# 0xMiden/miden-vm

Measured on AMD Instinct MI355X. Metric: trace rows/sec proved (2^20-row trace, 96-bit sec), higher is better.
Workload: dtype u64 (Goldilocks field, p = 2^64 - 2^32 + 1); 1 GPU; full proof of miden:20:51:8 (DummyMidenAir 2^20 x 51 + 8 EF aux), 96-bit production PCS params (blowup 8, FRI arity 4, 27 queries, PoW 4/12/16), Poseidon2 LMCS; trace resident in HBM, transcript on host; log_trace_rows=20, main_width=51, aux_width_ef=8, log_blowup=3, proof_bytes=137697, parallelism=1 GPU

## Files before the change

miden-vm_amd/csrc/deep.hip:

```cpp
#include "gl.cuh"
#include "kernels.hpp"

__global__ __launch_bounds__(256) void k_bary_weights(const u64* tw, int log_n, u64 g, e2 y0, e2 y1, u64* w0, u64* w1) {
  const size_t n = (size_t)1 << log_n;
  const size_t base = (size_t)blockIdx.x * 1024 + threadIdx.x;
  const size_t half = n >> 1;
  u64 xs[4], nrm[8], pre[8];
  e2 den[8];
#pragma unroll
  for (int k = 0; k < 4; k++) {
    size_t r = base + (size_t)k * 256;
    u64 x = 0;
    if (r < n) x = gl_mul(g, half ? (r < half ? tw[r] : gl_neg(tw[r - half])) : 1);
    xs[k] = x;
    den[2 * k] = e2_sub(y0, e2_make(x));
    den[2 * k + 1] = e2_sub(y1, e2_make(x));
  }
  u64 run = 1;
#pragma unroll
  for (int k = 0; k < 8; k++) {
    nrm[k] = gl_sub(gl_sqr(den[k].c0), gl_mul7(gl_sqr(den[k].c1)));
    pre[k] = run;
    run = gl_mul(run, nrm[k]);
  }
  u64 inv = gl_inv(run);
#pragma unroll
  for (int k = 7; k >= 0; k--) {
    u64 ni = gl_mul(inv, pre[k]);
    inv = gl_mul(inv, nrm[k]);
    size_t r = base + (size_t)(k >> 1) * 256;
    if (r < n) {
      u64 s = gl_mul(ni, xs[k >> 1]);
      u64* w = (k & 1) ? w1 : w0;
      w[2 * r] = gl_mul(den[k].c0, s);
      w[2 * r + 1] = gl_mul(gl_neg(den[k].c1), s);
    }
  }
}

static constexpr int OOD_ROWS_PER_BLOCK = 8192;
__global__ __launch_bounds__(256) void k_ood_partial(const u64* lde, int log_n, int log_blowup, const u64* w0, const u64* w1,
                                                     u64* partial, unsigned chunks) {
  __shared__ u64 red[4][256];
  const size_t n = (size_t)1 << log_n;
  const size_t col = blockIdx.y, chunk = blockIdx.x;
  const u64* f = lde + ((col << log_blowup) << log_n);
  const size_t r0 = chunk * OOD_ROWS_PER_BLOCK;
  const size_t r1 = r0 + OOD_ROWS_PER_BLOCK < n ? r0 + OOD_ROWS_PER_BLOCK : n;
  e2 a0 = e2_make(0), a1 = e2_make(0);
  for (size_t r = r0 + threadIdx.x; r < r1; r += 256) {
    u64 v = f[r];
    a0 = e2_add(a0, e2_mulf(e2{w0[2 * r], w0[2 * r + 1]}, v));
    a1 = e2_add(a1, e2_mulf(e2{w1[2 * r], w1[2 * r + 1]}, v));
  }
  red[0][threadIdx.x] = a0.c0; red[1][threadIdx.x] = a0.c1; red[2][threadIdx.x] = a1.c0; red[3][threadIdx.x] = a1.c1;
  __syncthreads();
  for (int s = 128; s > 0; s >>= 1) {
    if ((int)threadIdx.x < s) {
#pragma unroll
      for (int k = 0; k < 4; k++) red[k][threadIdx.x] = gl_add(red[k][threadIdx.x], red[k][threadIdx.x + s]);
    }
    __syncthreads();
  }
  if (threadIdx.x < 4) partial[(col * chunks + chunk) * 4 + threadIdx.x] = red[threadIdx.x][0];
}

void deep_ood_eval_batch(mh_ctx* c, std::vector<OodJob>& jobs, int log_blowup) {
  struct Weights {
    int log_n;
    size_t coset0;
    e2 y0, y1;
    DevBuf w0, w1;
  };
  std::vector<std::unique_ptr<Weights>> weights;
  struct Slot {
    size_t off = 0, ncol = 0;
    unsigned chunks = 0;
  };
  std::vector<Slot> slots(jobs.size());
  size_t total = 0;
  for (size_t k = 0; k < jobs.size(); k++) {
    OodJob& j = jobs[k];
    const LdeMatrix& m = *j.m;
    if (j.col_end > m.width) j.col_end = m.width;
    j.out0.assign(m.width, e2_make(0));
    j.out1.assign(m.width, e2_make(0));
    if (j.col_begin >= j.col_end) continue;
    const size_t n = (size_t)1 << m.log_n;
    slots[k].ncol = j.col_end - j.col_begin;
    slots[k].chunks = (unsigned)((n + OOD_ROWS_PER_BLOCK - 1) / OOD_ROWS_PER_BLOCK);
    slots[k].off = total;
    total += slots[k].ncol * slots[k].chunks * 4;
  }
  if (!total) return;
  DevBuf partial(total * 8), one;
  for (size_t k = 0; k < jobs.size(); k++) {
    if (!slots[k].ncol) continue;
    const OodJob& j = jobs[k];
    const LdeMatrix& m = *j.m;
    const int log_n = m.log_n;
    const size_t n = (size_t)1 << log_n;
    const u64 g = gl_mul(gl_lde_shift(log_n + log_blowup), gl_pow(gl_two_adic_generator(log_n + log_blowup), m.coset0));
    const u64* tw = log_n ? c->twiddles(log_n, false) : nullptr;
    if (!tw) {
      if (!one.p) {
        one.alloc(8);
        u64 v = 1;
        c->h2d(one.p, &v, 8);
      }
      tw = one.u();
    }
    ProfScope ps(c, "deep_ood_eval", (double)n * 8.0 * slots[k].ncol + 64.0 * n);
    Weights* w = nullptr;
    for (auto& cand : weights)
      if (cand->log_n == log_n && cand->coset0 == m.coset0 && e2_eq(cand->y0, j.y0) && e2_eq(cand->y1, j.y1)) w = cand.get();
    if (!w) {
      weights.emplace_back(new Weights{log_n, m.coset0, j.y0, j.y1, DevBuf(n * 16), DevBuf(n * 16)});
      w = weights.back().get();
      MH_LAUNCH(k_bary_weights, dim3((unsigned)((n + 1023) / 1024)), dim3(256), 0, c->stream, tw, log_n, g, j.y0, j.y1, w->w0.u(), w->w1.u());
    }
    MH_LAUNCH(k_ood_partial, dim3(slots[k].chunks, (unsigned)slots[k].ncol), dim3(256), 0, c->stream,
              m.lde.u() + ((j.col_begin << m.log_cosets) << log_n), log_n, m.log_cosets, w->w0.u(), w->w1.u(), partial.u() + slots[k].off,
              slots[k].chunks);
  }
  std::vector<u64> host(total);
  c->d2h(host.data(), partial.p, total * 8);
  for (size_t k = 0; k < jobs.size(); k++) {
    if (!slots[k].ncol) continue;
    OodJob& j = jobs[k];
    const LdeMatrix& m = *j.m;
    const int log_n = m.log_n;
    const size_t n = (size_t)1 << log_n;
    const u64 g = gl_mul(gl_lde_shift(log_n + log_blowup), gl_pow(gl_two_adic_generator(log_n + log_blowup), m.coset0));
    const u64 g_inv = gl_inv(g), n_inv = gl_inv((u64)n % GL_P);
    const e2 s0 = e2_mulf(e2_sub(e2_exp_pow2(e2_mulf(j.y0, g_inv), log_n), e2_make(1)), n_inv);
    const e2 s1 = e2_mulf(e2_sub(e2_exp_pow2(e2_mulf(j.y1, g_inv), log_n), e2_make(1)), n_inv);
    for (size_t col = 0; col < slots[k].ncol; col++) {
      e2 a0 = e2_make(0), a1 = e2_make(0);
      for (unsigned ch = 0; ch < slots[k].chunks; ch++) {
        const u64* p = host.data() + slots[k].off + (col * slots[k].chunks + ch) * 4;
        a0 = e2_add(a0, e2{p[0], p[1]});
        a1 = e2_add(a1, e2{p[2], p[3]});
      }
      j.out0[j.col_begin + col] = e2_mul(a0, s0);
      j.out1[j.col_begin + col] = e2_mul(a1, s1);
    }
  }
}
void deep_ood_eval_matrix(mh_ctx* c, const LdeMatrix& m, int log_blowup, e2 y0, e2 y1, std::vector<e2>& out0, std::vector<e2>& out1,
                          size_t col_begin, size_t col_end) {
  std::vector<OodJob> jobs(1);
  jobs[0].m = &m; jobs[0].y0 = y0; jobs[0].y1 = y1; jobs[0].col_begin = col_begin; jobs[0].col_end = col_end;
  deep_ood_eval_batch(c, jobs, log_blowup);
  out0.swap(jobs[0].out0);
  out1.swap(jobs[0].out1);
}

static constexpr int DEEP_MAX_MATS = 128;
static constexpr unsigned DEEP_FLUSH = 128;
#ifndef DEEP_UNROLL
#define DEEP_UNROLL 2
#endif
#ifndef DEEP_PTS_N
#define DEEP_PTS_N 1
#endif
static constexpr int DEEP_PTS = DEEP_PTS_N;
struct DeepMat {
  const u64* lde;
  u32 width, coef_off;
  int log_n;
};
struct DeepArgs {
  DeepMat m[DEEP_MAX_MATS];
  int n_mats, log_n, log_blowup;
  const u64* negc;
  const u64* tw;
  const u64* coset_x;
  e2 z0, z1, fred0, fred1, beta;
  u64* out;
};

template <bool PLANES>
__global__ __launch_bounds__(256) void k_deep_assemble(DeepArgs a) {
  const size_t N = (size_t)1 << a.log_n;
  const size_t j = blockIdx.y;
  const size_t base = (size_t)blockIdx.x * (256 * DEEP_PTS) + threadIdx.x;
  size_t r[DEEP_PTS];
#pragma unroll
  for (int k = 0; k < DEEP_PTS; k++) r[k] = base + (size_t)k * 256;
  e2 neg[DEEP_PTS];
  u64 w[DEEP_PTS][2][6];
#pragma unroll
  for (int k = 0; k < DEEP_PTS; k++) {
    neg[k] = e2_make(0);
#pragma unroll
    for (int e = 0; e < 2; e++)
#pragma unroll
      for (int i = 0; i < 6; i++) w[k][e][i] = 0;
  }
  auto flush = [&]() {
    const u64 C[6] = {1ULL, 1ULL << 22, 1ULL << 44, 1ULL << 32, 1ULL << 54, GL_EPS << 12};
#pragma unroll
    for (int k = 0; k < DEEP_PTS; k++) {
      u64 s0 = w[k][0][0], s1 = w[k][1][0];
#pragma unroll
      for (int i = 1; i < 6; i++) {
        s0 = gl_add(s0, gl_mul(w[k][0][i], C[i]));
        s1 = gl_add(s1, gl_mul(w[k][1][i], C[i]));
      }
      neg[k] = e2_add(neg[k], e2{s0, s1});
#pragma unroll
      for (int e = 0; e < 2; e++)
#pragma unroll
        for (int i = 0; i < 6; i++) w[k][e][i] = 0;
    }
  };
  u32 pending = 0;
#pragma unroll 1
  for (int mi = 0; mi < a.n_mats; mi++) {
    const DeepMat m = a.m[mi];
    const size_t nm_mask = ((size_t)1 << m.log_n) - 1;
    const u64* colp = m.lde + (j << m.log_n);
    const size_t cstride = (size_t)1 << (m.log_n + a.log_blowup);
#pragma unroll DEEP_UNROLL
    for (u32 cidx = 0; cidx < m.width; cidx++) {
      const u64 cf0 = a.negc[2 * (m.coef_off + cidx)], cf1 = a.negc[2 * (m.coef_off + cidx) + 1];
      u32 al[2][3];
#pragma unroll
      for (int i = 0; i < 3; i++) {
        al[0][i] = (u32)(cf0 >> (22 * i)) & 0x3FFFFFu;
        al[1][i] = (u32)(cf1 >> (22 * i)) & 0x3FFFFFu;
      }
#pragma unroll
      for (int k = 0; k < DEEP_PTS; k++) {
        if (r[k] < N) {
          const u64 v = colp[r[k] & nm_mask];
          const u32 v0 = (u32)v, v1 = (u32)(v >> 32);
#pragma unroll
          for (int e = 0; e < 2; e++) {
            w[k][e][0] += (u64)al[e][0] * v0;
            w[k][e][1] += (u64)al[e][1] * v0;
            w[k][e][2] += (u64)al[e][2] * v0;
            w[k][e][3] += (u64)al[e][0] * v1;
            w[k][e][4] += (u64)al[e][1] * v1;
            w[k][e][5] += (u64)al[e][2] * v1;
          }
        }
      }
      colp += cstride;
      if (++pending == DEEP_FLUSH) {
        flush();
        pending = 0;
      }
    }
  }
  flush();
  const size_t half = N >> 1;
  const u64 cx = a.coset_x[j];
  e2 den[2 * DEEP_PTS];
  u64 nrm[2 * DEEP_PTS], pre[2 * DEEP_PTS];
#pragma unroll
  for (int k = 0; k < DEEP_PTS; k++) {
    u64 x = 0;
    if (r[k] < N) x = gl_mul(cx, half ? (r[k] < half ? a.tw[r[k]] : gl_neg(a.tw[r[k] - half])) : 1);
    den[2 * k] = e2_sub(a.z0, e2_make(x));
    den[2 * k + 1] = e2_sub(a.z1, e2_make(x));
  }
  u64 run = 1;
#pragma unroll
  for (int k = 0; k < 2 * DEEP_PTS; k++) {
    nrm[k] = gl_sub(gl_sqr(den[k].c0), gl_mul7(gl_sqr(den[k].c1)));
    pre[k] = run;
    run = gl_mul(run, nrm[k]);
  }
  u64 inv = gl_inv(run);
  e2 qinv[2 * DEEP_PTS];
#pragma unroll
  for (int k = 2 * DEEP_PTS - 1; k >= 0; k--) {
    u64 ni = gl_mul(inv, pre[k]);
// ... 85 lines not shown
```

miden-vm_amd/csrc/ntt.hip:

```cpp
#include "ctx.hpp"
#include "gl.cuh"
#include "kernels.hpp"
#include "poseidon2_fast.cuh"
#include <utility>

#ifndef NTT_ASM_MUL
#define NTT_ASM_MUL 2
#endif
#if P2F_ASM && NTT_ASM_MUL == 1
#define NTT_MUL1 p2f_mul
#elif P2F_ASM && NTT_ASM_MUL == 2
#define NTT_MUL1 p2f_mul_nv
#else
#define NTT_MUL1 p2f_mul_c
#endif

static constexpr int NTT_TILE_LOG = 12;
static constexpr int NTT_TILE_LOG_BIG = 14;
static constexpr int NTT_THREADS = 256;
static int ntt_tile_log(int log_n) {
  static const int big_max = [] {
    const char* e = getenv("MH_NTT_BIG_MAX");
    return e ? atoi(e) : 22;
  }();
  return log_n > 20 && log_n <= big_max ? NTT_TILE_LOG_BIG : NTT_TILE_LOG;
}

static bool ntt_coef_rot(int log_n) {
  static const int on = [] { const char* e = getenv("MH_NTT_ROT"); return e ? atoi(e) : 1; }();
  return on && log_n >= NTT_TILE_LOG && ntt_tile_log(log_n) == NTT_TILE_LOG;
}

struct PowTable {
  u64 pw[32];
};
__global__ void k_fill_powers(u64* out, size_t n, PowTable t, u64 scale) {
  size_t k = blockIdx.x * (size_t)blockDim.x + threadIdx.x;
  if (k >= n) return;
  u64 r = scale;
  size_t e = k;
#pragma unroll 1
  for (int i = 0; e; i++, e >>= 1)
    if (e & 1) r = gl_mul(r, t.pw[i]);
  out[k] = r;
}

static void fill_powers(mh_ctx* c, u64* out, size_t n, u64 base, u64 scale) {
  PowTable t;
  u64 b = base;
  for (int i = 0; i < 32; i++) {
    t.pw[i] = b;
    b = gl_sqr(b);
  }
  if (n == 0) return;
  MH_LAUNCH(k_fill_powers, dim3((n + 255) / 256), dim3(256), 0, c->stream, out, n, t, scale);
}

const u64* mh_ctx::twiddles(int log_n, bool inverse) {
  auto& m = inverse ? tw_inv : tw_fwd;
  auto it = m.find(log_n);
  if (it != m.end()) return it->second.u();
  size_t half = log_n ? ((size_t)1 << (log_n - 1)) : 1;
  DevBuf b(half * 8);
  u64 w = gl_two_adic_generator(log_n);
  if (inverse) w = gl_inv(w);
  fill_powers(this, b.u(), half, w, 1);
  const u64* p = b.u();
  m[log_n] = std::move(b);
  return p;
}

__global__ __launch_bounds__(256) void k_transpose_rm_to_cm(const u64* __restrict__ in, u64* __restrict__ out, size_t n,
                                                           size_t w) {
  __shared__ u64 tile[32][33];
  size_t r0 = (size_t)blockIdx.x * 32, c0 = (size_t)blockIdx.y * 32;
  int tx = threadIdx.x & 31, ty = threadIdx.x >> 5;
  for (int k = ty; k < 32; k += 8) {
    size_t r = r0 + k, cc = c0 + tx;
    if (r < n && cc < w) tile[k][tx] = in[r * w + cc];
  }
  __syncthreads();
  for (int k = ty; k < 32; k += 8) {
    size_t cc = c0 + k, r = r0 + tx;
    if (r < n && cc < w) out[cc * n + r] = gl_canon(tile[tx][k]);
  }
}

void launch_transpose_rm_to_cm(mh_ctx* c, const u64* in, u64* out, size_t n, size_t w, hipStream_t stream) {
  dim3 grid((unsigned)((n + 31) / 32), (unsigned)((w + 31) / 32));
  MH_LAUNCH(k_transpose_rm_to_cm, grid, dim3(256), 0, stream ? stream : c->stream, in, out, n, w);
}

struct NttPassArgs {
  const u64* src;
  u64* dst;
  size_t src_col_stride, dst_col_stride, dst_z_stride;
  int log_n, s_lo, r_bits, cb;
  int dif;
  int canon_out;
  const u64* tw_round[4];
  const u64* scale_lo;
  const u64* scale_hi;
  int lb;
  size_t scale_lo_z, scale_hi_z;
  u32 n_z;
  const u64* scale_full;
  int col_fastest;
  size_t src_z_stride;
  int rot;
  int direct_first;
  u32 group_cols, group_z;
  const u64* step;
};

#if defined(__HIP_DEVICE_COMPILE__)
__device__ __forceinline__ u64 ntt_canon(u64 t) {
  const u64 u = t + GL_EPS;
  return u < t ? u : t;
}
__device__ __forceinline__ u64 ntt_add(u64 a, u64 t) {
  u64 s = a + t;
  s += (s < t) ? GL_EPS : 0;
  return s;
}
__device__ __forceinline__ u64 ntt_sub(u64 a, u64 t) {
  u64 d = a - t;
  d -= (a < t) ? GL_EPS : 0;
  return d;
}
__device__ __forceinline__ u64 ntt_mul_pow2(u64 x, int S) {
  const int q = S >> 5, r = S & 31;
  const u64 y01 = x << r;
  const u32 y2 = r ? (u32)(hi32(x) >> (32 - r)) : 0u;
  if (q == 0) {
    u64 v = (u64)y2 * 0xFFFFFFFFu + y01;
    v += (v < y01) ? GL_EPS : 0;
    return v;
  }
  if (q == 1) {
    const u64 a0 = (u64)lo32(y01) << 32;
    u64 v = (u64)hi32(y01) * 0xFFFFFFFFu + a0;
    v += (v < a0) ? GL_EPS : 0;
    u64 w = v - y2;
    w -= (v < (u64)y2) ? GL_EPS : 0;
    return w;
  }
  const u64 v = (u64)lo32(y01) * 0xFFFFFFFFu;
  const u64 b = ((u64)y2 << 32) | hi32(y01);
  u64 w = v - b;
  w -= (v < b) ? GL_EPS : 0;
  return w;
}
__device__ __forceinline__ void ntt_bfly_dit(u64& a, u64& b, int E) {
  const u64 t = ntt_canon(E % 96 ? ntt_mul_pow2(b, E % 96) : b);
  const u64 s = ntt_add(a, t), d = ntt_sub(a, t);
  if (E >= 96) { a = d; b = s; } else { a = s; b = d; }
}
__device__ __forceinline__ void ntt_bfly_dif(u64& a, u64& b, int E) {
  const u64 t = ntt_canon(b);
  const u64 s = ntt_add(a, t);
  const u64 d = E >= 96 ? ntt_sub(t, ntt_canon(a)) : ntt_sub(a, t);
  a = s;
  b = E % 96 ? ntt_mul_pow2(d, E % 96) : d;
}
#ifndef NTT_ASM_BFLY
#define NTT_ASM_BFLY 1
#endif
#define NTT_A asm volatile
#define NTT_DEAD(i, TXT_PRE, TXT_POST, ...)                                          \
  do {                                                                              \
    switch ((i) & 3) {                                                              \
      case 0: NTT_A(TXT_PRE "s[84:85]" TXT_POST : __VA_ARGS__ : "s84", "s85"); break; \
      case 1: NTT_A(TXT_PRE "s[86:87]" TXT_POST : __VA_ARGS__ : "s86", "s87"); break; \
      case 2: NTT_A(TXT_PRE "s[88:89]" TXT_POST : __VA_ARGS__ : "s88", "s89"); break; \
      default: NTT_A(TXT_PRE "s[90:91]" TXT_POST : __VA_ARGS__ : "s90", "s91"); break; \
    }                                                                               \
  } while (0)
template <int N>
__device__ __forceinline__ void ntt_reduce128N(u64 (&r)[N], const u64 (&lo)[N], const u32 (&h0)[N], const u32 (&h1)[N]) {
  u64 t[N], c1[N], bb[N], bw[N], c3[N], k3[N];
  u32 rl[N], rh[N];
#pragma unroll
  for (int i = 0; i < N; i++) NTT_A("v_mad_u64_u32 %0, %1, %2, -1, %3" : "=v"(t[i]), "=s"(c1[i]) : "v"(h0[i]), "v"(lo[i]));
#pragma unroll
  for (int i = 0; i < N; i++) NTT_A("v_subb_co_u32_e64 %0, %1, %2, %3, %4" : "=v"(rl[i]), "=s"(bb[i]) : "v"(lo32(t[i])), "v"(h1[i]), "s"(c1[i]));
#pragma unroll
  for (int i = 0; i < N; i++) NTT_DEAD(i, "v_addc_co_u32_e64 %0, ", ", %1, 0, %2", "=v"(rh[i]) : "v"(hi32(t[i])), "s"(c1[i]));
#pragma unroll
  for (int i = 0; i < N; i++) NTT_A("v_subb_co_u32_e64 %0, %1, %2, 0, %3" : "=v"(rh[i]), "=s"(bw[i]) : "0"(rh[i]), "s"(bb[i]));
#pragma unroll
  for (int i = 0; i < N; i++) NTT_A("v_addc_co_u32_e64 %0, %1, %2, 0, %3" : "=v"(rl[i]), "=s"(c3[i]) : "0"(rl[i]), "s"(bw[i]));
#pragma unroll
  for (int i = 0; i < N; i++) k3[i] = bw[i] & ~c3[i];
#pragma unroll
  for (int i = 0; i < N; i++) {
    NTT_DEAD(i, "v_subb_co_u32_e64 %0, ", ", %1, 0, %2", "=v"(rh[i]) : "0"(rh[i]), "s"(k3[i]));
    r[i] = ((u64)rh[i] << 32) | rl[i];
  }
}
template <int N>
__device__ __forceinline__ void ntt_bfly_tailN(u64 (&a)[N], u64 (&t)[N]) {
  u32 u0[N], u1[N], t0[N], t1[N], s0[N], s1[N], d0[N], d1[N];
  u64 c0[N], c1[N], ca[N], cb[N], bs[N], ks[N], b0[N], b1[N], cd[N], kd[N];
#pragma unroll
  for (int i = 0; i < N; i++) NTT_A("v_add_co_u32_e64 %0, %1, %2, -1" : "=v"(u0[i]), "=s"(c0[i]) : "v"(lo32(t[i])));
#pragma unroll
  for (int i = 0; i < N; i++) NTT_A("v_addc_co_u32_e64 %0, %1, %2, 0, %3" : "=v"(u1[i]), "=s"(c1[i]) : "v"(hi32(t[i])), "s"(c0[i]));
#pragma unroll
  for (int i = 0; i < N; i++) NTT_A("v_cndmask_b32_e64 %0, %1, %2, %3" : "=v"(t0[i]) : "v"(lo32(t[i])), "v"(u0[i]), "s"(c1[i]));
#pragma unroll
  for (int i = 0; i < N; i++) NTT_A("v_cndmask_b32_e64 %0, %1, %2, %3" : "=v"(t1[i]) : "v"(hi32(t[i])), "v"(u1[i]), "s"(c1[i]));
#pragma unroll
  for (int i = 0; i < N; i++) NTT_A("v_add_co_u32_e64 %0, %1, %2, %3" : "=v"(s0[i]), "=s"(ca[i]) : "v"(lo32(a[i])), "v"(t0[i]));
#pragma unroll
  for (int i = 0; i < N; i++) NTT_A("v_addc_co_u32_e64 %0, %1, %2, %3, %4" : "=v"(s1[i]), "=s"(cb[i]) : "v"(hi32(a[i])), "v"(t1[i]), "s"(ca[i]));
#pragma unroll
  for (int i = 0; i < N; i++) NTT_A("v_sub_co_u32_e64 %0, %1, %2, %3" : "=v"(d0[i]), "=s"(b0[i]) : "v"(lo32(a[i])), "v"(t0[i]));
#pragma unroll
  for (int i = 0; i < N; i++) NTT_A("v_subb_co_u32_e64 %0, %1, %2, %3, %4" : "=v"(d1[i]), "=s"(b1[i]) : "v"(hi32(a[i])), "v"(t1[i]), "s"(b0[i]));
#pragma unroll
  for (int i = 0; i < N; i++) NTT_A("v_subb_co_u32_e64 %0, %1, %2, 0, %3" : "=v"(s0[i]), "=s"(bs[i]) : "0"(s0[i]), "s"(cb[i]));
#pragma unroll
  for (int i = 0; i < N; i++) NTT_A("v_addc_co_u32_e64 %0, %1, %2, 0, %3" : "=v"(d0[i]), "=s"(cd[i]) : "0"(d0[i]), "s"(b1[i]));
#pragma unroll
  for (int i = 0; i < N; i++) {
    ks[i] = cb[i] & ~bs[i];
    kd[i] = b1[i] & ~cd[i];
  }
#pragma unroll
  for (int i = 0; i < N; i++) NTT_DEAD(i, "v_addc_co_u32_e64 %0, ", ", %1, 0, %2", "=v"(s1[i]) : "0"(s1[i]), "s"(ks[i]));
#pragma unroll
  for (int i = 0; i < N; i++) {
    NTT_DEAD(i + 2, "v_subb_co_u32_e64 %0, ", ", %1, 0, %2", "=v"(d1[i]) : "0"(d1[i]), "s"(kd[i]));
    a[i] = ((u64)s1[i] << 32) | s0[i];
    t[i] = ((u64)d1[i] << 32) | d0[i];
  }
}
template <int S>
__device__ __forceinline__ void ntt_shift_parts(u64 b, u64& lo, u32& h0, u32& h1) {
  constexpr int q = S >> 5, r = S & 31;
  const u32 b0 = lo32(b), b1 = hi32(b);
  const u32 y0 = r ? (b0 << r) : b0;
  const u32 y1 = r ? __builtin_amdgcn_alignbit(b1, b0, 32 - r) : b1;
  const u32 y2 = r ? (b1 >> (32 - r)) : 0u;
  if constexpr (q == 0) {
    lo = ((u64)y1 << 32) | y0; h0 = y2; h1 = 0;
  } else if constexpr (q == 1) {
    lo = (u64)y0 << 32; h0 = y1; h1 = y2;
  } else {
    lo = ((u64)(~y2) << 32) | 1u; h0 = y0; h1 = y1;
  }
}
__host__ __device__ constexpr int ntt_fwd_exp(int m, int e) { return (156 * (8 >> m) * (e & ((1 << m) - 1))) % 192; }
__host__ __device__ constexpr int ntt_bfly_lo(int m, int k) { return ((k >> m) << (m + 1)) | (k & ((1 << m) - 1)); }
__host__ __device__ constexpr bool ntt_bfly_shifted(int m, int k) { return (ntt_fwd_exp(m, ntt_bfly_lo(m, k)) % 96) != 0; }
__host__ __device__ constexpr int ntt_shift_slot(int m, int k) {
  int n = 0;
  for (int i = 0; i < k; i++) n += ntt_bfly_shifted(m, i);
  return n;
}
template <int H, int M, int K>
struct NttBfly {
  static constexpr int E = ntt_bfly_lo(M, K), EX = ntt_fwd_exp(M, E), SLOT = ntt_shift_slot(M, K);
  static constexpr bool SH = (EX % 96) != 0;
  __device__ __forceinline__ static void pre(const u64* x, u64* a, u64* t, u64* lo, u32* h0, u32* h1) {
    a[K] = x[E];
    if constexpr (SH) ntt_shift_parts<EX % 96>(x[E | (1 << M)], lo[SLOT], h0[SLOT], h1[SLOT]);
    else t[K] = x[E | (1 << M)];
    if constexpr (K + 1 < H) NttBfly<H, M, K + 1>::pre(x, a, t, lo, h0, h1);
  }
  __device__ __forceinline__ static void mid(u64* t, const u64* r) {
    if constexpr (SH) t[K] = r[SLOT];
    if constexpr (K + 1 < H) NttBfly<H, M, K + 1>::mid(t, r);
  }
  __device__ __forceinline__ static void post(u64* x, const u64* a, const u64* t) {
    if constexpr (EX >= 96) {
      x[E] = t[K];
      x[E | (1 << M)] = a[K];
    } else {
      x[E] = a[K];
      x[E | (1 << M)] = t[K];
    }
    if constexpr (K + 1 < H) NttBfly<H, M, K + 1>::post(x, a, t);
  }
};
#ifndef NTT_ILV
#define NTT_ILV 4
#endif
template <int N>
__device__ __forceinline__ void ntt_tail_split(u64 (&a)[N], u64 (&t)[N]) {
  if constexpr (N <= NTT_ILV) {
    ntt_bfly_tailN<N>(a, t);
  } else {
    constexpr int A = NTT_ILV, B = N - NTT_ILV;
    u64 a0[A], t0[A], a1[B], t1[B];
#pragma unroll
    for (int i = 0; i < A; i++) { a0[i] = a[i]; t0[i] = t[i]; }
#pragma unroll
    for (int i = 0; i < B; i++) { a1[i] = a[A + i]; t1[i] = t[A + i]; }
    ntt_bfly_tailN<A>(a0, t0);
    ntt_tail_split<B>(a1, t1);
#pragma unroll
    for (int i = 0; i < A; i++) { a[i] = a0[i]; t[i] = t0[i]; }
#pragma unroll
    for (int i = 0; i < B; i++) { a[A + i] = a1[i]; t[A + i] = t1[i]; }
  }
}
template <int N>
__device__ __forceinline__ void ntt_reduce_split(u64 (&r)[N], const u64 (&lo)[N], const u32 (&h0)[N], const u32 (&h1)[N]) {
  if constexpr (N <= NTT_ILV) {
    ntt_reduce128N<N>(r, lo, h0, h1);
  } else {
    constexpr int A = (N >= 2 * NTT_ILV || N - NTT_ILV >= 3) ? NTT_ILV : N - 3, B = N - A;
    u64 r0[A], lo0[A], r1[B], lo1[B];
    u32 p0[A], q0[A], p1[B], q1[B];
#pragma unroll
    for (int i = 0; i < A; i++) { lo0[i] = lo[i]; p0[i] = h0[i]; q0[i] = h1[i]; }
#pragma unroll
    for (int i = 0; i < B; i++) { lo1[i] = lo[A + i]; p1[i] = h0[A + i]; q1[i] = h1[A + i]; }
    ntt_reduce128N<A>(r0, lo0, p0, q0);
    ntt_reduce_split<B>(r1, lo1, p1, q1);
#pragma unroll
    for (int i = 0; i < A; i++) r[i] = r0[i];
#pragma unroll
    for (int i = 0; i < B; i++) r[A + i] = r1[i];
  }
}
template <int G, int M>
__device__ __forceinline__ void ntt_fwd_stage(u64 (&x)[1 << G]) {
  constexpr int H = 1 << (G - 1);
  constexpr int NS = ntt_shift_slot(M, H);
  u64 a[H], t[H];
  u64 lo[NS ? NS : 1], r[NS ? NS : 1];
  u32 h0[NS ? NS : 1], h1[NS ? NS : 1];
  NttBfly<H, M, 0>::pre(x, a, t, lo, h0, h1);
  if constexpr (NS > 0) {
    ntt_reduce_split<NS>(r, lo, h0, h1);
    NttBfly<H, M, 0>::mid(t, r);
  }
  ntt_tail_split<H>(a, t);
  NttBfly<H, M, 0>::post(x, a, t);
}
template <int G, int M = 0>
__device__ __forceinline__ void ntt_fwd_dft_asm(u64 (&x)[1 << G]) {
  if constexpr (M < G) {
    ntt_fwd_stage<G, M>(x);
    ntt_fwd_dft_asm<G, M + 1>(x);
  }
}

template <int G, bool INV>
__device__ __forceinline__ void ntt_dft_regs(u64 (&x)[1 << G], bool dif) {
#if P2F_ASM && NTT_ASM_BFLY
  if constexpr (!INV && G >= 3) {
    ntt_fwd_dft_asm<G>(x);
    return;
  }
#endif
  constexpr int W16 = INV ? 36 : 156;
  if (!dif) {
#pragma unroll
    for (int m = 0; m < G; m++)
#pragma unroll
      for (int e = 0; e < (1 << G); e++)
        if (!(e & (1 << m))) ntt_bfly_dit(x[e], x[e | (1 << m)], (W16 * (8 >> m) * (e & ((1 << m) - 1))) % 192);
  } else {
#pragma unroll
    for (int m = G - 1; m >= 0; m--)
#pragma unroll
      for (int e = 0; e < (1 << G); e++)
        if (!(e & (1 << m))) ntt_bfly_dif(x[e], x[e | (1 << m)], (W16 * (8 >> m) * (e & ((1 << m) - 1))) % 192);
  }
}
template <int K, int OFF>
__device__ __forceinline__ void ntt_tw_mul(u64* x, const u64* __restrict__ tw, int s, u32 gm) {
  if constexpr (K > 0) {
    constexpr int C = K >= 5 ? 5 : K;
    u64 a[C], b[C];
#pragma unroll
    for (int i = 0; i < C; i++) {
      a[i] = x[OFF + i];
      b[i] = (tw + ((size_t)(OFF + i - 1) << s))[gm];
    }
#if P2F_ASM && NTT_ASM_MUL == 1
    p2f_mulN<C>(a, a, b);
#else
#pragma unroll
    for (int i = 0; i < C; i++) a[i] = NTT_MUL1(a[i], b[i]);
#endif
#pragma unroll
    for (int i = 0; i < C; i++) x[OFF + i] = a[i];
    ntt_tw_mul<K - C, OFF + C>(x, tw, s, gm);
  }
}
#else
template <int K, int OFF>
__device__ void ntt_tw_mul(u64* x, const u64* __restrict__ tw, int s, u32 gm);
template <int G, bool INV>
__device__ void ntt_dft_regs(u64 (&x)[1 << G], bool dif);
__device__ u64 ntt_canon(u64 t);
__device__ u64 p2f_mul_c(u64 a, u64 b);
#endif

#ifndef NTT16_OCC
#define NTT16_OCC
#endif
#ifndef NTT_SWZ
#define NTT_SWZ 1
#endif
static size_t ntt_lds_bytes(int tile_log) {
  if (NTT_SWZ && tile_log == NTT_TILE_LOG) return ((size_t)1 << tile_log) * 8;
  return (((size_t)1 << tile_log) + ((size_t)1 << (tile_log - 4))) * 8;
}
template <bool SWZ>
__device__ __forceinline__ u32 ntt_pad(u32 l) {
  return SWZ ? (l ^ ((l >> 4) & 31u)) : (l + (l >> 4));
}

#define NTT_STORE(p, v) (*(p) = (v))
template <int G, bool INV, bool SWZ, int B0>
__device__ __forceinline__ void ntt_round(const NttPassArgs& a, u64* lds, int st, u32 tile_n, size_t lo0, u64* dst_direct,
                                          size_t gbase, const u64* __restrict__ tw, const u64* __restrict__ src_direct = nullptr,
                                          const u64* xin = nullptr) {
  const int b0 = B0 >= 0 ? B0 : st + a.cb, s = a.s_lo + st;
  const u32 cb_mask = (1u << a.cb) - 1;
  constexpr bool FAST = SWZ && B0 >= 0;
  for (u32 q = threadIdx.x; q < (tile_n >> G); q += blockDim.x) {
    const u32 low = q & ((1u << b0) - 1);
    const u32 l0 = ((q >> b0) << (b0 + G)) | low;
    const u32 gm = (((l0 >> a.cb) & ((1u << st) - 1)) << a.s_lo) | ((u32)lo0 << a.cb) | (l0 & cb_mask);
    const u32 p0 = ntt_pad<SWZ>(l0);
    char* const ldsb = reinterpret_cast<char*>(lds);
    const u32 pb = p0 * 8u, pb1 = (p0 ^ 16u) * 8u;
    auto slot = [&](int e) -> u64* {
      if constexpr (FAST && B0 == 8) return reinterpret_cast<u64*>(ldsb + ((e & 1) ? pb1 : pb) + ((u32)e << 11));
      else if constexpr (FAST) return reinterpret_cast<u64*>(ldsb + (pb ^ (ntt_pad<true>((u32)e << B0) * 8u)));
      else return lds + (SWZ ? (p0 ^ ntt_pad<true>((u32)e << b0)) : ntt_pad<false>(l0 | ((u32)e << b0)));
    };
    u64 x[1 << G];
    if (xin) {
#pragma unroll
      for (int e = 0; e < (1 << G); e++) x[e] = xin[e];
    } else if (src_direct) {
      const u32 six = (u32)(gbase | ((size_t)(l0 >> a.cb) << a.s_lo) | (l0 & cb_mask));
#pragma unroll
      for (int e = 0; e < (1 << G); e++) x[e] = (src_direct + ((size_t)e << s))[six];
    } else {
#pragma unroll
    for (int e = 0; e < (1 << G); e++) x[e] = *slot(e);
    }
    if (!INV && s > 0) ntt_tw_mul<(1 << G) - 1, 1>(x, tw, s, gm);
    ntt_dft_regs<G, INV>(x, INV);
    if (INV && s > 0) ntt_tw_mul<(1 << G) - 1, 1>(x, tw, s, gm);
    if (INV && dst_direct && a.rot && b0 == 0 && G == 4) {
      const u32 rix = (u32)gbase + (l0 >> 4);
#pragma unroll
      for (int e = 0; e < (1 << G); e++) NTT_STORE((dst_direct + ((size_t)e << 8)) + rix, a.canon_out ? ntt_canon(x[e]) : x[e]);
    } else if (dst_direct) {
      const u32 tix = (u32)(gbase | ((size_t)(l0 >> a.cb) << a.s_lo) | (l0 & cb_mask));
      if (a.canon_out) {
#pragma unroll
        for (int e = 0; e < (1 << G); e++) NTT_STORE((dst_direct + ((size_t)e << s)) + tix, ntt_canon(x[e]));
      } else {
#pragma unroll
        for (int e = 0; e < (1 << G); e++) NTT_STORE((dst_direct + ((size_t)e << s)) + tix, x[e]);
      }
    } else {
#pragma unroll
      for (int e = 0; e < (1 << G); e++) *slot(e) = x[e];
    }
  }
}

template <bool INV, int THREADS, int MODE = 0>
__global__ __launch_bounds__(THREADS) NTT16_OCC void k_ntt16_pass(NttPassArgs a) {
  extern __shared__ u64 lds[];
  constexpr bool SWZ = NTT_SWZ && THREADS == NTT_THREADS;
  const int tile_log = a.r_bits + a.cb;
  const u32 tile_n = 1u << tile_log;
  const u32 cb_mask = (1u << a.cb) - 1;
  const u32 tile = a.col_fastest ? blockIdx.y : blockIdx.x;
  const u32 col_id = a.col_fastest ? blockIdx.x : blockIdx.y;
  const int lo_bits = a.s_lo - a.cb;
  const size_t lo0 = tile & ((1u << lo_bits) - 1);
  const size_t hi = tile >> lo_bits;
  const size_t gbase = (hi << (a.s_lo + a.r_bits)) | (lo0 << a.cb);
  const u64* src0 = a.src + (size_t)col_id * a.src_col_stride;
  u64 raw[MODE == 1 ? 16 : 1];
  for (u32 z = 0; z < a.n_z; z++) {
  const u32 zc = blockIdx.z * a.n_z + z;
  const u32 srow = a.group_cols ? (col_id / a.group_cols) * a.group_z + zc : zc;
  u64* dst = a.dst + (size_t)col_id * a.dst_col_stride + (size_t)zc * a.dst_z_stride;
  const u64* src = src0 + (size_t)zc * a.src_z_stride;
  if (z) __syncthreads();

  constexpr int LOG_T = THREADS == 256 ? 8 : 10;
  const bool direct_first = MODE == 0 && THREADS == NTT_THREADS && a.direct_first && tile_n == 16u * THREADS;
  if (direct_first) {
  } else if (tile_n == 16u * THREADS && a.cb <= LOG_T) {
    const u32 tid = threadIdx.x;
    const u32 g0 = (u32)(gbase | ((size_t)(tid >> a.cb) << a.s_lo) | (tid & cb_mask));
    const int shg = LOG_T - a.cb + a.s_lo;
    const u32 p0 = ntt_pad<SWZ>(tid);
    if constexpr (MODE == 1) {
      if (z == 0) {
#pragma unroll
// ... 426 lines not shown
```

Before: 24.19 million trace rows/s.

## Group columns in OOD evaluation kernel and reduce chunk partials on device

Adds a column-grouped OOD partial kernel that loads each barycentric weight pair once and reuses it across 8 columns. It processes 4 rows per thread per iteration with vectorized weight loads and reduces with wave shuffles instead of a shared-memory tree. A second small kernel sums the chunk partials on the GPU, so only one value per column is copied back rather than every chunk partial. The old per-column path stays behind an environment variable. This costs more registers per thread and fewer blocks per column.

```diff
diff --git a/miden-vm_amd/csrc/deep.hip b/miden-vm_amd/csrc/deep.hip
--- a/miden-vm_amd/csrc/deep.hip
+++ b/miden-vm_amd/csrc/deep.hip
@@ -65,7 +65,94 @@
   if (threadIdx.x < 4) partial[(col * chunks + chunk) * 4 + threadIdx.x] = red[threadIdx.x][0];
 }
 
+#ifndef OOD_GROUP_COLS
+#define OOD_GROUP_COLS 8
+#endif
+static constexpr int OOD_GROUP_ROWS = 4;
+static constexpr int OOD_GROUP_ROWS_PER_BLOCK = 2048;
+template <int G>
+__global__ __launch_bounds__(256) void k_ood_partial_group(const u64* lde, int log_n, int log_blowup, const u64* w0, const u64* w1,
+                                                           u64* partial, unsigned chunks, unsigned ncol) {
+  __shared__ u64 red[4][G * 4];
+  const size_t n = (size_t)1 << log_n;
+  const size_t chunk = blockIdx.x, c0 = (size_t)blockIdx.y * G;
+  const unsigned gc = ncol - (unsigned)c0 < (unsigned)G ? ncol - (unsigned)c0 : (unsigned)G;
+  const size_t cstride = (size_t)1 << (log_n + log_blowup);
+  const u64* f = lde + c0 * cstride;
+  const size_t r0 = chunk * OOD_GROUP_ROWS_PER_BLOCK;
+  const size_t r1 = r0 + OOD_GROUP_ROWS_PER_BLOCK < n ? r0 + OOD_GROUP_ROWS_PER_BLOCK : n;
+  e2 a0[G], a1[G];
+#pragma unroll
+  for (int g = 0; g < G; g++) a0[g] = a1[g] = e2_make(0);
+  for (size_t rb = r0 + threadIdx.x; rb < r1; rb += 256 * OOD_GROUP_ROWS) {
+    e2 x0[OOD_GROUP_ROWS], x1[OOD_GROUP_ROWS];
+#pragma unroll
+    for (int k = 0; k < OOD_GROUP_ROWS; k++) {
+      const size_t r = rb + (size_t)k * 256;
+      x0[k] = x1[k] = e2_make(0);
+      if (r < r1) {
+        const ulonglong2 p0 = *reinterpret_cast<const ulonglong2*>(w0 + 2 * r), p1 = *reinterpret_cast<const ulonglong2*>(w1 + 2 * r);
+        x0[k] = e2{p0.x, p0.y};
+        x1[k] = e2{p1.x, p1.y};
+      }
+    }
+#pragma unroll
+    for (int g = 0; g < G; g++) {
+      if ((unsigned)g < gc) {
+        u64 v[OOD_GROUP_ROWS];
+#pragma unroll
+        for (int k = 0; k < OOD_GROUP_ROWS; k++) {
+          const size_t r = rb + (size_t)k * 256;
+          v[k] = r < r1 ? f[(size_t)g * cstride + r] : 0;
+        }
+#pragma unroll
+        for (int k = 0; k < OOD_GROUP_ROWS; k++) {
+          a0[g] = e2_add(a0[g], e2_mulf(x0[k], v[k]));
+          a1[g] = e2_add(a1[g], e2_mulf(x1[k], v[k]));
+        }
+      }
+    }
+  }
+  const unsigned lane = threadIdx.x & 63, wave = threadIdx.x >> 6;
+#pragma unroll
+  for (int g = 0; g < G; g++) {
+    u64 s[4] = {a0[g].c0, a0[g].c1, a1[g].c0, a1[g].c1};
+#pragma unroll
+    for (int k = 0; k < 4; k++) {
+#pragma unroll
+      for (int off = 32; off > 0; off >>= 1) s[k] = gl_add(s[k], (u64)__shfl_down((unsigned long long)s[k], off, 64));
+      if (lane == 0) red[wave][g * 4 + k] = s[k];
+    }
+  }
+  __syncthreads();
+  if (threadIdx.x < gc * 4) {
+    const unsigned t = threadIdx.x;
+    const u64 s = gl_add(gl_add(red[0][t], red[1][t]), gl_add(red[2][t], red[3][t]));
+    partial[((c0 + (t >> 2)) * chunks + chunk) * 4 + (t & 3)] = s;
+  }
+}
+
+__global__ __launch_bounds__(64) void k_ood_sum_chunks(const u64* partial, const u64* where, u64* sums) {
+  const size_t col = blockIdx.x;
+  const u64* p = partial + where[2 * col];
+  const unsigned chunks = (unsigned)where[2 * col + 1];
+  u64 s[4] = {0, 0, 0, 0};
+  for (unsigned ch = threadIdx.x; ch < chunks; ch += 64) {
+#pragma unroll
+    for (int k = 0; k < 4; k++) s[k] = gl_add(s[k], p[(size_t)ch * 4 + k]);
+  }
+#pragma unroll
+  for (int k = 0; k < 4; k++) {
+#pragma unroll
+    for (int off = 32; off > 0; off >>= 1) s[k] = gl_add(s[k], (u64)__shfl_down((unsigned long long)s[k], off, 64));
+    if (threadIdx.x == 0) sums[col * 4 + k] = s[k];
+  }
+}
+
 void deep_ood_eval_batch(mh_ctx* c, std::vector<OodJob>& jobs, int log_blowup) {
+  const char* per_env = getenv("MH_OOD_PER_COLUMN");
+  const bool per_column = per_env && atoi(per_env);
+  const size_t rows_per_block = per_column ? OOD_ROWS_PER_BLOCK : OOD_GROUP_ROWS_PER_BLOCK;
   struct Weights {
     int log_n;
     size_t coset0;
@@ -74,11 +161,11 @@
   };
   std::vector<std::unique_ptr<Weights>> weights;
   struct Slot {
-    size_t off = 0, ncol = 0;
+    size_t off = 0, ncol = 0, col0 = 0;
     unsigned chunks = 0;
   };
   std::vector<Slot> slots(jobs.size());
-  size_t total = 0;
+  size_t total = 0, total_cols = 0;
   for (size_t k = 0; k < jobs.size(); k++) {
     OodJob& j = jobs[k];
     const LdeMatrix& m = *j.m;
@@ -88,9 +175,11 @@
     if (j.col_begin >= j.col_end) continue;
     const size_t n = (size_t)1 << m.log_n;
     slots[k].ncol = j.col_end - j.col_begin;
-    slots[k].chunks = (unsigned)((n + OOD_ROWS_PER_BLOCK - 1) / OOD_ROWS_PER_BLOCK);
+    slots[k].chunks = (unsigned)((n + rows_per_block - 1) / rows_per_block);
     slots[k].off = total;
+    slots[k].col0 = total_cols;
     total += slots[k].ncol * slots[k].chunks * 4;
+    total_cols += slots[k].ncol;
   }
   if (!total) return;
   DevBuf partial(total * 8), one;
@@ -110,7 +199,8 @@
       }
       tw = one.u();
     }
-    ProfScope ps(c, "deep_ood_eval", (double)n * 8.0 * slots[k].ncol + 64.0 * n);
+    const size_t groups = (slots[k].ncol + OOD_GROUP_COLS - 1) / OOD_GROUP_COLS;
+    ProfScope ps(c, "deep_ood_eval", (double)n * 8.0 * slots[k].ncol + 32.0 * n + 32.0 * n * (per_column ? 1 : groups));
     Weights* w = nullptr;
     for (auto& cand : weights)
       if (cand->log_n == log_n && cand->coset0 == m.coset0 && e2_eq(cand->y0, j.y0) && e2_eq(cand->y1, j.y1)) w = cand.get();
@@ -119,12 +209,36 @@
       w = weights.back().get();
       MH_LAUNCH(k_bary_weights, dim3((unsigned)((n + 1023) / 1024)), dim3(256), 0, c->stream, tw, log_n, g, j.y0, j.y1, w->w0.u(), w->w1.u());
     }
-    MH_LAUNCH(k_ood_partial, dim3(slots[k].chunks, (unsigned)slots[k].ncol), dim3(256), 0, c->stream,
-              m.lde.u() + ((j.col_begin << m.log_cosets) << log_n), log_n, m.log_cosets, w->w0.u(), w->w1.u(), partial.u() + slots[k].off,
-              slots[k].chunks);
-  }
-  std::vector<u64> host(total);
-  c->d2h(host.data(), partial.p, total * 8);
+    const u64* cols = m.lde.u() + ((j.col_begin << m.log_cosets) << log_n);
+    if (per_column)
+      MH_LAUNCH(k_ood_partial, dim3(slots[k].chunks, (unsigned)slots[k].ncol), dim3(256), 0, c->stream, cols, log_n, m.log_cosets,
+                w->w0.u(), w->w1.u(), partial.u() + slots[k].off, slots[k].chunks);
+    else
+      MH_LAUNCH(k_ood_partial_group<OOD_GROUP_COLS>, dim3(slots[k].chunks, (unsigned)groups), dim3(256), 0, c->stream, cols, log_n,
+                m.log_cosets, w->w0.u(), w->w1.u(), partial.u() + slots[k].off, slots[k].chunks, (unsigned)slots[k].ncol);
+  }
+  std::vector<u64> host(per_column ? total : total_cols * 4);
+  if (per_column) {
+    c->d2h(host.data(), partial.p, total * 8);
+  } else {
+    std::vector<u64> where(2 * total_cols);
+    for (size_t k = 0; k < jobs.size(); k++)
+      for (size_t col = 0; col < slots[k].ncol; col++) {
+        where[2 * (slots[k].col0 + col)] = slots[k].off + col * slots[k].chunks * 4;
+        where[2 * (slots[k].col0 + col) + 1] = slots[k].chunks;
+      }
+    DevBuf dwhere(where.size() * 8), sums(total_cols * 4 * 8);
+    c->h2d(dwhere.p, where.data(), where.size() * 8);
+    {
+      ProfScope ps(c, "deep_ood_sum", (double)total * 8.0 + 32.0 * total_cols);
+      MH_LAUNCH(k_ood_sum_chunks, dim3((unsigned)total_cols), dim3(64), 0, c->stream, partial.u(), dwhere.u(), sums.u());
+    }
+    c->d2h(host.data(), sums.p, total_cols * 4 * 8);
+    for (size_t k = 0; k < jobs.size(); k++) {
+      slots[k].off = slots[k].col0 * 4;
+      slots[k].chunks = slots[k].ncol ? 1 : 0;
+    }
+  }
   for (size_t k = 0; k < jobs.size(); k++) {
     if (!slots[k].ncol) continue;
     OodJob& j = jobs[k];
```

Result: no change. 24.18 million trace rows/s (-0.1%).

## Use lazy 96-bit wide representation for in-register NTT butterflies

Applied to the files above, without the earlier changes.

Adds a new default in-register DFT path that holds values as three 32-bit limbs with a bias, so butterflies need only add/sub with carry chains and shift-based twiddles. Full modular reduction is deferred to a single fold at the end, with selective pre-folds where growth would overflow. This now also covers the inverse transform and small G, which previously used the canonical C path. The aim is fewer reductions per butterfly, at the cost of higher register pressure from the extra limb and correctness risk in the bias and overflow bookkeeping.

```diff
diff --git a/miden-vm_amd/csrc/ntt.hip b/miden-vm_amd/csrc/ntt.hip
--- a/miden-vm_amd/csrc/ntt.hip
+++ b/miden-vm_amd/csrc/ntt.hip
@@ -164,7 +164,7 @@
   b = E % 96 ? ntt_mul_pow2(d, E % 96) : d;
 }
 #ifndef NTT_ASM_BFLY
-#define NTT_ASM_BFLY 1
+#define NTT_ASM_BFLY 2
 #endif
 #define NTT_A asm volatile
 #define NTT_DEAD(i, TXT_PRE, TXT_POST, ...)                                          \
@@ -349,9 +349,157 @@
   }
 }
 
+#define NTT_WIDE_FOLD_FWD 0x22000000u
+#define NTT_WIDE_FOLD_INV 0x000C0200u
+#if P2F_ASM && NTT_ASM_BFLY == 2
+struct NttW {
+  u32 w0, w1, w2;
+};
+__device__ __forceinline__ NttW ntt_w_from(u64 x) { return NttW{lo32(x), hi32(x), 0u}; }
+__device__ __forceinline__ NttW ntt_w_bias(NttW a) {
+  const u64 zlo = 0xC000000040000000ULL, lo = (((u64)a.w1 << 32) | a.w0) + zlo;
+  return NttW{lo32(lo), hi32(lo), a.w2 + 0x3FFFFFFFu + (lo < zlo ? 1u : 0u)};
+}
+__device__ __forceinline__ NttW ntt_w_sub1(NttW a, NttW b) {
+  NttW d;
+  u64 b0, b1, b2;
+  asm("v_sub_co_u32_e64 %0, %1, %2, %3" : "=v"(d.w0), "=s"(b0) : "v"(a.w0), "v"(b.w0));
+  asm("s_nop 1\n\tv_subb_co_u32_e64 %0, %1, %2, %3, %4" : "=v"(d.w1), "=s"(b1) : "v"(a.w1), "v"(b.w1), "s"(b0));
+  asm("s_nop 1\n\tv_subb_co_u32_e64 %0, %1, %2, %3, %4" : "=v"(d.w2), "=s"(b2) : "v"(a.w2), "v"(b.w2), "s"(b1));
+  return d;
+}
+__device__ __forceinline__ u64 ntt_w_fold1(NttW v) {
+  u64 t, c, r, d0;
+  u32 m;
+  const u64 lo = ((u64)v.w1 << 32) | v.w0;
+  asm("v_mad_u64_u32 %0, %1, %2, -1, %3" : "=v"(t), "=s"(c) : "v"(v.w2), "v"(lo));
+  asm("s_nop 1\n\tv_cndmask_b32_e64 %0, 0, -1, %1" : "=v"(m) : "s"(c));
+  asm("v_mad_u64_u32 %0, %1, %2, 1, %3" : "=v"(r), "=s"(d0) : "v"(m), "v"(t));
+  return r;
+}
+template <int N>
+__device__ __forceinline__ void ntt_w_foldN(u64 (&r)[N], const u32 (&w0)[N], const u32 (&w1)[N], const u32 (&w2)[N]) {
+  u64 t[N], c[N];
+  u32 m[N];
+#pragma unroll
+  for (int i = 0; i < N; i++) NTT_A("v_mad_u64_u32 %0, %1, %2, -1, %3" : "=v"(t[i]), "=s"(c[i]) : "v"(w2[i]), "v"(((u64)w1[i] << 32) | w0[i]));
+  if constexpr (N < 3) NTT_A("s_nop 1");
+#pragma unroll
+  for (int i = 0; i < N; i++) NTT_A("v_cndmask_b32_e64 %0, 0, -1, %1" : "=v"(m[i]) : "s"(c[i]));
+#pragma unroll
+  for (int i = 0; i < N; i++) NTT_DEAD(i, "v_mad_u64_u32 %0, ", ", %1, 1, %2", "=v"(r[i]) : "v"(m[i]), "v"(t[i]));
+}
+template <int N>
+__device__ __forceinline__ void ntt_w_bflyN(NttW (&s)[N], NttW (&d)[N], const NttW (&a)[N], const NttW (&t)[N], const NttW (&p)[N],
+                                            const NttW (&q)[N]) {
+  u64 ca[N], cb[N], ba[N], bb[N];
+#pragma unroll
+  for (int i = 0; i < N; i++) NTT_A("v_add_co_u32_e64 %0, %1, %2, %3" : "=v"(s[i].w0), "=s"(ca[i]) : "v"(a[i].w0), "v"(t[i].w0));
+#pragma unroll
+  for (int i = 0; i < N; i++) NTT_A("v_sub_co_u32_e64 %0, %1, %2, %3" : "=v"(d[i].w0), "=s"(ba[i]) : "v"(p[i].w0), "v"(q[i].w0));
+  if constexpr (N == 1) NTT_A("s_nop 0");
+#pragma unroll
+  for (int i = 0; i < N; i++) NTT_A("v_addc_co_u32_e64 %0, %1, %2, %3, %4" : "=v"(s[i].w1), "=s"(cb[i]) : "v"(a[i].w1), "v"(t[i].w1), "s"(ca[i]));
+#pragma unroll
+  for (int i = 0; i < N; i++) NTT_A("v_subb_co_u32_e64 %0, %1, %2, %3, %4" : "=v"(d[i].w1), "=s"(bb[i]) : "v"(p[i].w1), "v"(q[i].w1), "s"(ba[i]));
+  if constexpr (N == 1) NTT_A("s_nop 0");
+#pragma unroll
+  for (int i = 0; i < N; i++) NTT_DEAD(i, "v_addc_co_u32_e64 %0, ", ", %1, %2, %3", "=v"(s[i].w2) : "v"(a[i].w2), "v"(t[i].w2), "s"(cb[i]));
+#pragma unroll
+  for (int i = 0; i < N; i++) NTT_DEAD(i + 2, "v_subb_co_u32_e64 %0, ", ", %1, %2, %3", "=v"(d[i].w2) : "v"(p[i].w2), "v"(q[i].w2), "s"(bb[i]));
+}
+__device__ __forceinline__ NttW ntt_w_shl(NttW b, int S) {
+  const int q = S >> 5, r = S & 31;
+  const u32 y0 = r ? (b.w0 << r) : b.w0;
+  const u32 y1 = r ? __builtin_amdgcn_alignbit(b.w1, b.w0, 32 - r) : b.w1;
+  const u32 y2 = r ? __builtin_amdgcn_alignbit(b.w2, b.w1, 32 - r) : b.w2;
+  if (q == 0) return NttW{y0, y1, y2};
+  const u32 ys = (u32)((int)y2 >> 31);
+  if (q == 1) {
+    u64 t, c, d0;
+    u32 h;
+    const u64 a0 = (u64)y0 << 32;
+    asm("v_mad_u64_u32 %0, %1, %2, -1, %3" : "=v"(t), "=s"(c) : "v"(y1), "v"(a0));
+    asm("s_nop 1\n\tv_addc_co_u32_e64 %0, %1, 0, 0, %2" : "=v"(h), "=s"(d0) : "s"(c));
+    return ntt_w_sub1(NttW{lo32(t), hi32(t), h}, NttW{y2, ys, ys});
+  }
+  const u64 pe = (u64)y0 * 0xFFFFFFFFu;
+  return ntt_w_sub1(NttW{lo32(pe), hi32(pe), 0u}, NttW{y1, y2, ys});
+}
+template <int G, bool INV, int M, int K0, int N>
+__device__ __forceinline__ void ntt_w_stage_part(u32 (&v0)[1 << G], u32 (&v1)[1 << G], u32 (&v2)[1 << G]) {
+  constexpr int W16 = INV ? 36 : 156;
+  constexpr u32 FOLD = INV ? NTT_WIDE_FOLD_INV : NTT_WIDE_FOLD_FWD;
+  NttW a[N], t[N], p[N], q[N], s[N], d[N];
+#pragma unroll
+  for (int i = 0; i < N; i++) {
+    const int e = ntt_bfly_lo(M, K0 + i), f = e | (1 << M), j = e & ((1 << M) - 1);
+    const int E = (W16 * (8 >> M) * j) % 192, S = E % 96;
+    const bool pre = (FOLD >> (8 * M + j)) & 1u;
+    a[i] = NttW{v0[e], v1[e], v2[e]};
+    t[i] = NttW{v0[f], v1[f], v2[f]};
+    if (!INV) {
+      if (S) t[i] = ntt_w_shl(pre ? ntt_w_from(ntt_w_fold1(ntt_w_bias(t[i]))) : t[i], S);
+      p[i] = a[i];
+      q[i] = t[i];
+    } else {
+      p[i] = E >= 96 ? t[i] : a[i];
+      q[i] = E >= 96 ? a[i] : t[i];
+    }
+  }
+  ntt_w_bflyN<N>(s, d, a, t, p, q);
+#pragma unroll
+  for (int i = 0; i < N; i++) {
+    const int e = ntt_bfly_lo(M, K0 + i), f = e | (1 << M), j = e & ((1 << M) - 1);
+    const int E = (W16 * (8 >> M) * j) % 192, S = E % 96;
+    const bool pre = (FOLD >> (8 * M + j)) & 1u;
+    NttW lo = s[i], hi = d[i];
+    if (!INV) {
+      if (E >= 96) { lo = d[i]; hi = s[i]; }
+    } else if (S) {
+      hi = ntt_w_shl(pre ? ntt_w_from(ntt_w_fold1(ntt_w_bias(hi))) : hi, S);
+    }
+    v0[e] = lo.w0; v1[e] = lo.w1; v2[e] = lo.w2;
+    v0[f] = hi.w0; v1[f] = hi.w1; v2[f] = hi.w2;
+  }
+}
+template <int G, bool INV, int I = 0>
+__device__ __forceinline__ void ntt_w_stages(u32 (&v0)[1 << G], u32 (&v1)[1 << G], u32 (&v2)[1 << G]) {
+  if constexpr (I < G) {
+    constexpr int M = INV ? G - 1 - I : I, H = 1 << (G - 1), N = H < NTT_ILV ? H : NTT_ILV;
+    ntt_w_stage_part<G, INV, M, 0, N>(v0, v1, v2);
+    if constexpr (H > N) ntt_w_stage_part<G, INV, M, N, H - N>(v0, v1, v2);
+    ntt_w_stages<G, INV, I + 1>(v0, v1, v2);
+  }
+}
+template <int G, bool INV>
+__device__ __forceinline__ void ntt_dft_wide(u64 (&x)[1 << G]) {
+  u32 v0[1 << G], v1[1 << G], v2[1 << G];
+#pragma unroll
+  for (int e = 0; e < (1 << G); e++) { v0[e] = lo32(x[e]); v1[e] = hi32(x[e]); v2[e] = 0u; }
+  const NttW z = ntt_w_bias(NttW{v0[0], v1[0], 0u});
+  v0[0] = z.w0; v1[0] = z.w1; v2[0] = z.w2;
+  ntt_w_stages<G, INV>(v0, v1, v2);
+  constexpr int NF = (1 << G) < NTT_ILV ? (1 << G) : NTT_ILV;
+#pragma unroll
+  for (int c = 0; c < (1 << G); c += NF) {
+    u64 r[NF];
+    u32 f0[NF], f1[NF], f2[NF];
+#pragma unroll
+    for (int i = 0; i < NF; i++) { f0[i] = v0[c + i]; f1[i] = v1[c + i]; f2[i] = v2[c + i]; }
+    ntt_w_foldN<NF>(r, f0, f1, f2);
+#pragma unroll
+    for (int i = 0; i < NF; i++) x[c + i] = r[i];
+  }
+}
+#endif
+
 template <int G, bool INV>
 __device__ __forceinline__ void ntt_dft_regs(u64 (&x)[1 << G], bool dif) {
-#if P2F_ASM && NTT_ASM_BFLY
+#if P2F_ASM && NTT_ASM_BFLY == 2
+  ntt_dft_wide<G, INV>(x);
+  return;
+#elif P2F_ASM && NTT_ASM_BFLY
   if constexpr (!INV && G >= 3) {
     ntt_fwd_dft_asm<G>(x);
     return;
```

Result: faster. 23.80 million trace rows/s before, 24.32 million trace rows/s after, median of 6 (+2.2%).
